# Membrizard/ml_conformer_generator

Hardware: NVIDIA B200
Metric: generated mols/sec (100 EGNN steps + GCN, <=39 atoms) (higher is better)
Workload: dtype fp16

## Files before the change

ml_conformer_generator_b200/csrc/mlcg_api.cu:

```cuda
#include <algorithm>
#include <cstddef>
#include <cstdlib>
#include <cstring>
#include <map>
#include <string>
#include <vector>

#include "mlcg.h"
#include "mlcg_kernels.cuh"
#include "mlcg_tc.cuh"
#include "mlcg_tc3.cuh"
#include "mlcg_shape.cuh"
#include "mlcg_ifm.cuh"

using namespace mlcg;

namespace {

struct Wt {
  float* d = nullptr;
  int rows = 0, cols = 0;
};

struct DevBuf {
// ... 94 lines not shown
#define KCHECK()                                 \
  do {                                           \
    h->launches++;                               \
    CK(cudaGetLastError());                      \
  } while (0)
#define FAIL(code, msg) \
  do {                  \
    h->err = (msg);     \
    return (code);      \
  } while (0)

static thread_local std::string g_create_err;

enum { BD_START = -1, BD_PREPARE = 0, BD_PQ = 1, BD_EDGE_GCL = 2, BD_EDGE_EQUIV = 3, BD_FIXUP = 4, BD_MLP1 = 5, BD_MLP2 = 6,
       BD_READOUT = 7, BD_NCLASS = 8 };
static void bd_mark(mlcg_handle* h, int cls, cudaStream_t st) {
  if (!h->bd_on) return;
  cudaEvent_t e;
  if (cudaEventCreate(&e) != cudaSuccess) return;
  cudaEventRecord(e, st);
  h->bd_ev.emplace_back(cls, e);
}

template <int kMode, int BN, int kEpi>
static cudaError_t launch_gemm(const GemmArgs& a, int n_mtiles, int n_ntiles, cudaStream_t st) {
  static bool attr_set = false;
  if (!attr_set) {
    cudaError_t e = cudaFuncSetAttribute(k_tc_gemm<kMode, BN, kEpi>, cudaFuncAttributeMaxDynamicSharedMemorySize,
                                         GemmCfg<BN>::SMEM_BYTES);
    if (e != cudaSuccess) return e;
    attr_set = true;
  }
  static int num_sms = 0;
  if (num_sms == 0) {
    int dev = 0;
    cudaGetDevice(&dev);
    cudaDeviceGetAttribute(&num_sms, cudaDevAttrMultiProcessorCount, dev);
    if (num_sms <= 0) num_sms = 148;
  }
  GemmArgs b = a;
  b.n_mtiles = n_mtiles;
  b.n_ntiles = n_ntiles;
  k_tc_gemm<kMode, BN, kEpi><<<std::min(n_mtiles * n_ntiles, num_sms), GEMM_THREADS, GemmCfg<BN>::SMEM_BYTES, st>>>(b);
  return cudaGetLastError();
}
template <int BN, int kEpi>
static cudaError_t launch_gemm_mode(int mode, const GemmArgs& a, int n_mtiles, int n_ntiles, cudaStream_t st) {
  if (mode == PREC_FP16) return launch_gemm<PREC_FP16, BN, kEpi>(a, n_mtiles, n_ntiles, st);
  return mode == PREC_BF16 ? launch_gemm<PREC_BF16, BN, kEpi>(a, n_mtiles, n_ntiles, st)
                           : launch_gemm<PREC_TF32, BN, kEpi>(a, n_mtiles, n_ntiles, st);
}
template <int kMode, bool kEquiv, bool kPair, bool kDistF32 = false, bool kProf = false>
static cudaError_t launch_edge(const EdgeArgs& a, int grid, cudaStream_t st) {
  static bool attr_set = false;
  if (!attr_set) {
    cudaError_t e = cudaFuncSetAttribute(k_tc_edge<kMode, kEquiv, kPair, kDistF32, kProf>, cudaFuncAttributeMaxDynamicSharedMemorySize,
                                         EdgeSmemT<kMode>::ALLOC);
    if (e != cudaSuccess) return e;
    attr_set = true;
  }
  cudaLaunchConfig_t cfg{};
  cfg.gridDim = dim3(grid);
  cfg.blockDim = dim3(EDGE_THREADS);
  cfg.dynamicSmemBytes = EdgeSmemT<kMode>::ALLOC;
  cfg.stream = st;
  cudaLaunchAttribute attr[1];
  attr[0].id = cudaLaunchAttributeClusterDimension;
  attr[0].val.clusterDim.x = kPair ? 2 : 1;
  attr[0].val.clusterDim.y = 1;
  attr[0].val.clusterDim.z = 1;
  cfg.attrs = attr;
  cfg.numAttrs = 1;
  return cudaLaunchKernelEx(&cfg, k_tc_edge<kMode, kEquiv, kPair, kDistF32, kProf>, a);
// ... 612 lines not shown
      return (u + 0x7fffu + ((u >> 16) & 1u)) >> 16;
    };
    for (int k2 = 0; k2 < HP / 2; ++k2) {
      a.wcd_h[4 * (k2 / 2) + (k2 & 1)] = bf(L.h_wc[2 * k2]) | (bf(L.h_wc[2 * k2 + 1]) << 16);
      a.wcd_h[4 * (k2 / 2) + 2 + (k2 & 1)] = bf(L.h_wd[2 * k2]) | (bf(L.h_wd[2 * k2 + 1]) << 16);
    }
  }
  a.att_bias = L.att_bias;
  a.agg_op = h->agg_op.as<uint8_t>();
  a.agg_chunks = h->kc448();
  a.prof = nullptr;
  return a;
}

static int egnn_forward_tc(mlcg_handle* h, cudaStream_t st) {
  const int mode = h->precision, kc = h->kc448();
  const int grid_e = edge_grid(h);
  auto gemm_pq = [&](const LayerW& L) -> cudaError_t {
    GemmArgs a{};
    a.a0 = h->h_op.as<uint8_t>(); a.a0_chunks = kc; a.a0_per_tile = kc; a.n_kc = kc;
    a.w = L.w1ab_op.as<uint8_t>(); a.bias = L.bias_pq.as<float>(); a.m_rows = h->pl->M;
    a.out_f32 = h->pq.as<float>(); a.ldo = 2 * HP; a.n_valid = 2 * HP; a.rowscale = nullptr; a.relu = 0;
    a.out_scale = act_scale(mode);
    if (mode == PREC_FP16) return launch_gemm<PREC_FP16, HP, EPI_BF16>(a, h->pl->n_mtiles, 2, st);
    if (mode == PREC_BF16) return launch_gemm<PREC_BF16, HP, EPI_BF16>(a, h->pl->n_mtiles, 2, st);
    return launch_gemm<PREC_TF32, HP, EPI_F32>(a, h->pl->n_mtiles, 2, st);
  };
  float* xa = h->xa.as<float>();
  float* xb = h->xb.as<float>();
  CK(gemm_pq(h->layers[0]));
  h->launches++;
  bd_mark(h, BD_PQ, st);
  for (int l = 0; l < 27; ++l) {
    const LayerW& L = h->layers[l];
    const int blk = l / 3;
    const float* x_cur = (blk & 1) ? xb : xa;
    float* x_next = (blk & 1) ? xa : xb;
    EdgeArgs ea = edge_args(h, L, x_cur, x_next);
    CK(launch_edge_mode(mode, L.equiv, ea, grid_e, st));
    h->launches++;
    bd_mark(h, L.equiv ? BD_EDGE_EQUIV : BD_EDGE_GCL, st);
    CK(launch_edge_fixup(h, mode, L.equiv, ea, st));
    bd_mark(h, BD_FIXUP, st);
    if (!L.equiv) {
      GemmArgs a{};
      a.a0 = h->h_op.as<uint8_t>(); a.a0_chunks = kc; a.a0_per_tile = kc;
      a.a1 = h->agg_op.as<uint8_t>(); a.a1_per_tile = kc; a.n_kc = 2 * kc;
      a.w = L.w3_op.as<uint8_t>(); a.bias = L.b3p.as<float>(); a.m_rows = h->pl->M;
      a.out_op = h->t_op.as<uint8_t>(); a.out_op_chunks = kc; a.out_scale = op_scale(mode);
      CK((launch_gemm_mode<HP, EPI_SILU_OP>(mode, a, h->pl->n_mtiles, 1, st)));
      h->launches++;
      bd_mark(h, BD_MLP1, st);
      GemmArgs b{};
      b.a0 = h->t_op.as<uint8_t>(); b.a0_chunks = kc; b.a0_per_tile = kc; b.n_kc = kc;
      b.w = L.w4_op.as<uint8_t>(); b.bias = L.b4p.as<float>(); b.m_rows = h->pl->M;
      b.out_op = h->h_op.as<uint8_t>(); b.out_op_chunks = kc; b.resid = h->h_res.as<float>(); b.ldr = 0;
      b.out_scale = op_scale(mode);
      CK((launch_gemm_mode<HP, EPI_RESID_OP>(mode, b, h->pl->n_mtiles, 1, st)));
      h->launches++;
      bd_mark(h, BD_MLP2, st);
    }
    if (l + 1 < 27) {
      CK(gemm_pq(h->layers[l + 1]));
      h->launches++;
      bd_mark(h, BD_PQ, st);
    }
  }
  return MLCG_OK;
}

static int simt_gemm(mlcg_handle* h, const float* A, int lda, const float* W, int ldw, const float* bias, float* C, int ldc,
                     int M, int N, int K, int flags, const float* rowscale, cudaStream_t st) {
  if (M <= 0) return MLCG_OK;
  dim3 grid((N + 63) / 64, (M + 63) / 64);
  k_simt_gemm<<<grid, 256, 0, st>>>(A, lda, W, ldw, bias, rowscale, C, ldc, M, N, K, flags);
  KCHECK();
  return MLCG_OK;
}

static int egnn_forward_simt(mlcg_handle* h, cudaStream_t st) {
  float* xa = h->xa.as<float>();
// ... 704 lines not shown
  KCHECK();
  return MLCG_OK;
}

extern "C" int mlcg_ifm_merge_inputs(mlcg_handle* h, const float* x_gen, const int32_t* cls_gen, const float* shift,
                                     const float* rot, const float* ff_x, const float* ff_h, int n_ff, int B, int Ng, int N,
                                     float* z_known, float* fixed_mask, void* stream) {
  if (!h) return MLCG_E_ARG;
  if (!x_gen || !cls_gen || !shift || !rot || !ff_x || !ff_h || !z_known || !fixed_mask || B <= 0 || n_ff <= 0 || Ng <= 0 ||
      N < n_ff || N > 64)
    FAIL(MLCG_E_ARG, "ifm_merge_inputs: bad argument");
  k_ifm_merge_inputs<<<B, 64, 0, (cudaStream_t)stream>>>(x_gen, cls_gen, shift, rot, ff_x, ff_h, n_ff, Ng, N, z_known, fixed_mask);
  KCHECK();
  return MLCG_OK;
}

extern "C" int mlcg_gemm_phase_profile(mlcg_handle* h, int which, double* out, void* stream) {
  if (!h || !out) return MLCG_E_ARG;
  if (!h->egnn_loaded || !h->batch_set || h->precision == PREC_FP32_SIMT || which < 0 || which > 2)
    FAIL(MLCG_E_STATE, "gemm_phase_profile: needs a tensor-core precision, weights, a batch and which in 0..2");
  cudaStream_t st = (cudaStream_t)stream;
  const int mode = h->precision, kc = h->kc448();
  const LayerW& L = h->layers[0];
  const int grid = std::min(h->pl->n_mtiles * (which == 0 ? 2 : 1), h->num_sms);
  DevBuf buf;
  CK(buf.ensure((size_t)grid * 8 * sizeof(long long)));
  CK(cudaMemsetAsync(buf.p, 0, (size_t)grid * 8 * sizeof(long long), st));
  GemmArgs a{};
  a.prof = buf.as<long long>();
  a.m_rows = h->pl->M;
  a.out_scale = (which == 0) ? act_scale(mode) : op_scale(mode);
  cudaEvent_t e0, e1;
  CK(cudaEventCreate(&e0));
  CK(cudaEventCreate(&e1));
  CK(cudaEventRecord(e0, st));
  if (which == 0) {
    a.a0 = h->h_op.as<uint8_t>(); a.a0_chunks = kc; a.a0_per_tile = kc; a.n_kc = kc;
    a.w = L.w1ab_op.as<uint8_t>(); a.bias = L.bias_pq.as<float>();
    a.out_f32 = h->pq.as<float>(); a.ldo = 2 * HP; a.n_valid = 2 * HP;
    if (mode == PREC_FP16) CK((launch_gemm<PREC_FP16, HP, EPI_BF16>(a, h->pl->n_mtiles, 2, st)));
    else if (mode == PREC_BF16) CK((launch_gemm<PREC_BF16, HP, EPI_BF16>(a, h->pl->n_mtiles, 2, st)));
    else CK((launch_gemm<PREC_TF32, HP, EPI_F32>(a, h->pl->n_mtiles, 2, st)));
  } else if (which == 1) {
    a.a0 = h->h_op.as<uint8_t>(); a.a0_chunks = kc; a.a0_per_tile = kc;
    a.a1 = h->agg_op.as<uint8_t>(); a.a1_per_tile = kc; a.n_kc = 2 * kc;
    a.w = L.w3_op.as<uint8_t>(); a.bias = L.b3p.as<float>();
    a.out_op = h->t_op.as<uint8_t>(); a.out_op_chunks = kc;
    CK((launch_gemm_mode<HP, EPI_SILU_OP>(mode, a, h->pl->n_mtiles, 1, st)));
  } else {
    a.a0 = h->t_op.as<uint8_t>(); a.a0_chunks = kc; a.a0_per_tile = kc; a.n_kc = kc;
    a.w = L.w4_op.as<uint8_t>(); a.bias = L.b4p.as<float>();
    a.out_op = h->h_op.as<uint8_t>(); a.out_op_chunks = kc; a.resid = h->h_res.as<float>(); a.ldr = 0;
    CK((launch_gemm_mode<HP, EPI_RESID_OP>(mode, a, h->pl->n_mtiles, 1, st)));
  }
  CK(cudaEventRecord(e1, st));
  h->launches++;
  std::vector<long long> host((size_t)grid * 8);
  CK(cudaMemcpyAsync(host.data(), buf.p, host.size() * sizeof(long long), cudaMemcpyDeviceToHost, st));
  CK(cudaStreamSynchronize(st));
  float ms = 0.f;
  cudaEventElapsedTime(&ms, e0, e1);
  cudaEventDestroy(e0);
  cudaEventDestroy(e1);
  buf.release();
  for (int k = 0; k < 8; ++k) out[k] = 0.0;
  for (int b = 0; b < grid; ++b)
    for (int k = 0; k < 7; ++k) out[k] += (double)host[(size_t)b * 8 + k] / grid;
  out[7] = ms;
  return MLCG_OK;
}

extern "C" int mlcg_test_gemm(mlcg_handle* h, int mode, int bn, const float* a, const float* w, const float* bias, float* c,
                              int M, int N, int K, void* stream) {
  if (!h) return MLCG_E_ARG;
  if ((mode != PREC_TF32 && mode != PREC_BF16 && mode != PREC_FP16) || (bn != 448 && bn != 256) || !a || !w || !bias || !c || M <= 0 || N <= 0 || K <= 0)
    FAIL(MLCG_E_ARG, "test_gemm: bad argument");
  if (N % 4 != 0) FAIL(MLCG_E_ARG, "test_gemm: N must be a multiple of 4");
  cudaStream_t st = (cudaStream_t)stream;
  const int kc = (K + epc(mode) - 1) / epc(mode);
  const int mt = (M + TILE_M - 1) / TILE_M, nt = (N + bn - 1) / bn;
  CK(h->tg_a.ensure((size_t)mt * kc * A_CHUNK_BYTES));
  CK(h->tg_w.ensure((size_t)nt * kc * bn * CHUNK_BYTES));
  CK(h->tg_b.ensure((size_t)nt * bn * 4));
  CK(cudaMemsetAsync(h->tg_b.p, 0, (size_t)nt * bn * 4, st));
  CK(cudaMemcpyAsync(h->tg_b.p, bias, (size_t)N * 4, cudaMemcpyDeviceToDevice, st));
  const long long pieces = (long long)M * kc * 8;
  if (mode == PREC_FP16) k_rowmajor_to_op<PREC_FP16><<<(unsigned)((pieces + 255) / 256), 256, 0, st>>>(a, K, M, K, h->tg_a.as<uint8_t>(), kc);
  else if (mode == PREC_BF16) k_rowmajor_to_op<PREC_BF16><<<(unsigned)((pieces + 255) / 256), 256, 0, st>>>(a, K, M, K, h->tg_a.as<uint8_t>(), kc);
  else k_rowmajor_to_op<PREC_TF32><<<(unsigned)((pieces + 255) / 256), 256, 0, st>>>(a, K, M, K, h->tg_a.as<uint8_t>(), kc);
  KCHECK();
  PackArgs pa{};
  pa.src = w; pa.ld = K; pa.n_real = N; pa.bn = bn; pa.n_kc = kc; pa.seg_len = kc * epc(mode); pa.kreal0 = K;
  pa.bias = nullptr; pa.bias_k = -1; pa.dst = h->tg_w.as<uint8_t>();
  CK(launch_pack(mode, pa, nt, st));
  h->launches++;
  GemmArgs g{};
  g.a0 = h->tg_a.as<uint8_t>(); g.a0_chunks = kc; g.a0_per_tile = kc; g.n_kc = kc;
  g.w = h->tg_w.as<uint8_t>(); g.bias = h->tg_b.as<float>(); g.m_rows = M;
  g.out_f32 = c; g.ldo = N; g.n_valid = N; g.rowscale = nullptr; g.relu = 0;
  if (bn == 448) CK((launch_gemm_mode<448, EPI_F32>(mode, g, mt, nt, st)));
  else CK((launch_gemm_mode<256, EPI_F32>(mode, g, mt, nt, st)));
  h->launches++;
  return MLCG_OK;
}
```

ml_conformer_generator_b200/csrc/mlcg_tc.cuh:

```cuda
#pragma once
#include "mlcg_common.cuh"

namespace mlcg {

enum GemmEpi { EPI_F32 = 0, EPI_SILU_OP = 1, EPI_RESID_OP = 2, EPI_BF16 = 3 };

struct GemmArgs {
  const uint8_t* a0;
  const uint8_t* a1;
  int a0_chunks;
  int a0_per_tile;
  int a1_per_tile;
  int n_kc;
  const uint8_t* w;
  const float* bias;
  int m_rows;
  float* out_f32;
  int ldo;
  int n_valid;
  const float* rowscale;
  int relu;
  uint8_t* out_op;
  int out_op_chunks;
  float* resid;
  int ldr;
  float out_scale;
  int n_mtiles, n_ntiles;
  long long* prof;
};

template <int BN>
struct GemmCfg {
  static constexpr int NSTAGE = (BN == 448) ? 3 : 4;
  static constexpr int NPER = (BN == 448) ? 224 : BN;
  static constexpr int NH = BN / NPER;
  static constexpr int STAGE_BYTES = A_CHUNK_BYTES + BN * CHUNK_BYTES;
  static constexpr int TMEM_COLS = (BN > 256) ? 512 : 256;
  static constexpr int BIAS_OFF = NSTAGE * STAGE_BYTES + 256;
  static constexpr int SMEM_BYTES = NSTAGE * STAGE_BYTES + 1024  + 256  + 2 * BN * 4;
};

#ifndef MLCG_GEMM_NSUB
#define MLCG_GEMM_NSUB 2
#endif
constexpr int GEMM_NSUB = MLCG_GEMM_NSUB;
constexpr int GEMM_THREADS = 64 + 128 * GEMM_NSUB;

template <int kMode, int BN, int kEpi>
__global__ void __launch_bounds__(GEMM_THREADS, 1) k_tc_gemm(const GemmArgs p) {
  using Cfg = GemmCfg<BN>;
  constexpr bool kFast = is16(kMode);
  extern __shared__ uint8_t smem_raw[];
  const uint32_t base = (smem_u32(smem_raw) + 1023u) & ~1023u;
  uint8_t* gen_base = smem_raw + (base - smem_u32(smem_raw));
  const uint32_t bar0 = base + Cfg::NSTAGE * Cfg::STAGE_BYTES;
  auto full_bar = [&](int s) { return bar0 + 8u * s; };
  auto empty_bar = [&](int s) { return bar0 + 8u * (Cfg::NSTAGE + s); };
  const uint32_t dfull_bar = bar0 + 8u * (2 * Cfg::NSTAGE);
  uint32_t* tmem_slot = reinterpret_cast<uint32_t*>(gen_base + Cfg::NSTAGE * Cfg::STAGE_BYTES + 8 * (2 * Cfg::NSTAGE + 2));

  const uint32_t epi_done = dfull_bar + 8u;
  const int warp = threadIdx.x >> 5, lane = threadIdx.x & 31;
  const int n_tiles = p.n_mtiles * p.n_ntiles;

  if (threadIdx.x == 0) {
    for (int s = 0; s < Cfg::NSTAGE; ++s) {
      mbar_init(full_bar(s), 1);
      mbar_init(empty_bar(s), 1);
    }
    mbar_init(dfull_bar, 1);
    mbar_init(epi_done, 4 * GEMM_NSUB);
    fence_barrier_init();
  }
  if (warp == 1) tmem_alloc<Cfg::TMEM_COLS>(smem_u32(tmem_slot));
// ... 67 lines not shown
#pragma unroll
            for (int ks = 0; ks < 4; ++ks)
              umma<kMode>(tmem_base + nh * Cfg::NPER, adesc + 2 * ks, bdesc + 2 * ks, idesc, (kc | ks) != 0);
          }
          umma_commit(empty_bar(sl));
        }
        umma_commit(dfull_bar);
      }
      if (p.prof) {
        p.prof[(size_t)blockIdx.x * 8 + 1] = w_ops;
        p.prof[(size_t)blockIdx.x * 8 + 2] = w_epi;
        p.prof[(size_t)blockIdx.x * 8 + 5] = tl;
        p.prof[(size_t)blockIdx.x * 8 + 6] = clock64() - t_start;
      }
    }
  } else {
   int tl = 0;
   long long w_acc = 0, t_epi = 0;
   for (int tile = blockIdx.x; tile < n_tiles; tile += gridDim.x, ++tl) {
    const int mt = tile / p.n_ntiles, nt = tile - mt * p.n_ntiles;
    float* bias_s = reinterpret_cast<float*>(gen_base + Cfg::BIAS_OFF) + (tl & 1) * BN;
    for (int i = threadIdx.x - 64; i < BN; i += GEMM_THREADS - 64) bias_s[i] = p.bias[nt * BN + i];
    named_bar_sync(1, GEMM_THREADS - 64);
    const int q = warp & 3;
    const int row = q * 32 + lane;
    const int grow = mt * TILE_M + row;
    const bool rvalid = grow < p.m_rows;
    const long long pc0 = p.prof ? clock64() : 0;
    mbar_wait(dfull_bar, (uint32_t)(tl & 1));
    tc_fence_after();
    const long long pc1 = p.prof ? clock64() : 0;
    const uint32_t trow = tmem_base + ((uint32_t)(q * 32) << 16);
    if constexpr (kEpi == EPI_F32) {
      float rs = 1.0f;
      if (p.rowscale != nullptr && rvalid) rs = p.rowscale[grow];
      for (int c0 = ((warp - 2) >> 2) * 32; c0 < BN; c0 += 32 * GEMM_NSUB) {
        float v[32];
        tmem_ld32(trow + c0, v);
        tmem_wait_ld();
        const int gcol = nt * BN + c0;
        if (rvalid) {
          const float4* b4 = reinterpret_cast<const float4*>(bias_s + c0);
          float* orow = p.out_f32 + (size_t)grow * p.ldo + gcol;
#pragma unroll
          for (int e = 0; e < 32; e += 4) {
            const float4 b = b4[e >> 2];
            float4 o;
            o.x = fmaf(rs, b.x, v[e + 0]);
            o.y = fmaf(rs, b.y, v[e + 1]);
            o.z = fmaf(rs, b.z, v[e + 2]);
            o.w = fmaf(rs, b.w, v[e + 3]);
            if (p.relu) {
              o.x = fmaxf(o.x, 0.f); o.y = fmaxf(o.y, 0.f); o.z = fmaxf(o.z, 0.f); o.w = fmaxf(o.w, 0.f);
            }
            if (gcol + e + 3 < p.n_valid) {
              *reinterpret_cast<float4*>(orow + e) = o;
            } else {
              if (gcol + e + 0 < p.n_valid) orow[e + 0] = o.x;
              if (gcol + e + 1 < p.n_valid) orow[e + 1] = o.y;
              if (gcol + e + 2 < p.n_valid) orow[e + 2] = o.z;
            }
          }
        }
      }
    } else {
      constexpr int EPC = epc(kMode);
      constexpr int UNIT = EPC / 32;
      constexpr int NBLK = BN / EPC;
      const int sub = (warp - 2) >> 2;
      const int n_my = ((NBLK - sub + GEMM_NSUB - 1) / GEMM_NSUB) * UNIT;
      auto group_c0 = [&](int k) { return ((sub + GEMM_NSUB * (k / UNIT)) * UNIT + (k % UNIT)) * 32; };
      uint8_t* stg = gen_base + (sub * 4 + q) * 4096;
      const int crow = lane >> 3, cpiece = lane & 7;
      auto stg_at = [&](int r, int pc) { return stg + r * 128 + ((pc ^ (r & 7)) << 4); };
      const int row0 = mt * TILE_M + q * 32;
      uint32_t ow[32];
      [[maybe_unused]] uint4 rnext[8];
      if constexpr (kEpi == EPI_RESID_OP) {
        if (n_my > 0) {
          const uint4* nblk = reinterpret_cast<const uint4*>(p.resid + hres_index(row0, nt * BN + group_c0(0), 0));
#pragma unroll
          for (int i = 0; i < 8; ++i) rnext[i] = nblk[i * 32 + lane];
        }
      }
      for (int gk = 0; gk < n_my; ++gk) {
        const int c0 = group_c0(gk);
        float v[32];
        tmem_ld32(trow + c0, v);
        tmem_wait_ld();
        const int gcol = nt * BN + c0;
        const float4* b4 = reinterpret_cast<const float4*>(bias_s + c0);
        if constexpr (kEpi == EPI_RESID_OP) {
          float* rblk = p.resid + hres_index(row0, gcol, 0);
#pragma unroll
          for (int i = 0; i < 8; ++i) *reinterpret_cast<uint4*>(stg_at(4 * i + crow, cpiece)) = rnext[i];
          if (gk + 1 < n_my) {
            const uint4* nblk = reinterpret_cast<const uint4*>(p.resid + hres_index(row0, nt * BN + group_c0(gk + 1), 0));
#pragma unroll
            for (int i = 0; i < 8; ++i) rnext[i] = nblk[i * 32 + lane];
          }
          __syncwarp();
#pragma unroll
          for (int e = 0; e < 32; e += 4) {
            const float4 b = b4[e >> 2];
            float4 h = *reinterpret_cast<const float4*>(stg_at(lane, e >> 2));
            h.x += v[e + 0] + b.x;
            h.y += v[e + 1] + b.y;
            h.z += v[e + 2] + b.z;
            h.w += v[e + 3] + b.w;
            *reinterpret_cast<float4*>(stg_at(lane, e >> 2)) = h;
            v[e + 0] = h.x; v[e + 1] = h.y; v[e + 2] = h.z; v[e + 3] = h.w;
          }
          __syncwarp();
#pragma unroll
          for (int i = 0; i < 8; ++i)
            if (row0 + 4 * i + crow < p.m_rows)
              reinterpret_cast<uint4*>(rblk)[i * 32 + lane] = *reinterpret_cast<const uint4*>(stg_at(4 * i + crow, cpiece));
          __syncwarp();
        } else {
#pragma unroll
          for (int e = 0; e < 32; e += 4) {
            const float4 b = b4[e >> 2];
            if constexpr (kEpi == EPI_SILU_OP) {
              v[e + 0] = silu<kFast>(v[e + 0] + b.x); v[e + 1] = silu<kFast>(v[e + 1] + b.y);
              v[e + 2] = silu<kFast>(v[e + 2] + b.z); v[e + 3] = silu<kFast>(v[e + 3] + b.w);
            } else {
              v[e + 0] += b.x; v[e + 1] += b.y; v[e + 2] += b.z; v[e + 3] += b.w;
            }
          }
        }
        if constexpr (kMode == PREC_FP16) {
#pragma unroll
          for (int e = 0; e < 32; ++e) v[e] *= p.out_scale;
        }
        const bool flush = (EPC == 32) || ((c0 & 32) != 0);
        if constexpr (EPC == 32) {
#pragma unroll
          for (int j = 0; j < 32; ++j) ow[j] = f32_to_tf32(v[j]);
        } else {
          if ((c0 & 32) == 0) {
#pragma unroll
            for (int j = 0; j < 16; ++j) ow[j] = pack_h2<kMode>(v[2 * j], v[2 * j + 1]);
          } else {
#pragma unroll
            for (int j = 0; j < 16; ++j) ow[16 + j] = pack_h2<kMode>(v[2 * j], v[2 * j + 1]);
          }
        }
        if (flush) {
#pragma unroll
          for (int pc = 0; pc < 8; ++pc)
            *reinterpret_cast<uint4*>(stg_at(lane, pc)) = make_uint4(ow[4 * pc], ow[4 * pc + 1], ow[4 * pc + 2], ow[4 * pc + 3]);
          __syncwarp();
          const int cb0 = nt * BN + (c0 / EPC) * EPC;
          if constexpr (kEpi == EPI_BF16) {
            uint8_t* obase = reinterpret_cast<uint8_t*>(p.out_f32) + (size_t)cb0 * 2 + cpiece * 16;
#pragma unroll
            for (int i = 0; i < 8; ++i) {
              const int r = 4 * i + crow;
              if (row0 + r < p.m_rows)
                *reinterpret_cast<uint4*>(obase + (size_t)(row0 + r) * p.ldo * 2) = *reinterpret_cast<const uint4*>(stg_at(r, cpiece));
            }
          } else {
            uint8_t* dst = p.out_op + ((size_t)mt * p.out_op_chunks + cb0 / EPC) * A_CHUNK_BYTES + q * 4096;
#pragma unroll
            for (int i = 0; i < 8; ++i)
              if (row0 + 4 * i + crow < p.m_rows)
                reinterpret_cast<uint4*>(dst)[i * 32 + lane] = reinterpret_cast<const uint4*>(stg)[i * 32 + lane];
          }
          __syncwarp();
        }
      }
    }
    tc_fence_before();
    __syncwarp();
    if (lane == 0) mbar_arrive(epi_done);
    if (p.prof) { w_acc += pc1 - pc0; t_epi += clock64() - pc1; }
   }
   if (p.prof && warp == 2 && lane == 0) {
     p.prof[(size_t)blockIdx.x * 8 + 3] = w_acc;
     p.prof[(size_t)blockIdx.x * 8 + 4] = t_epi;
   }
  }
  tc_fence_before();
  __syncthreads();
  if (warp == 1) tmem_dealloc<Cfg::TMEM_COLS>(tmem_base);
}

constexpr int EDGE_MAXG = 12;
constexpr int EDGE_MAXN = 39;
constexpr int EDGE_WSLOT = 224 * CHUNK_BYTES;
constexpr int EDGE_NW = 3;
constexpr int EDGE_NWMAX = EDGE_NW;
constexpr int EDGE_NA = 2;
#ifndef MLCG_EDGE_EARLY
#define MLCG_EDGE_EARLY 2
// ... 762 lines not shown
```

ml_conformer_generator_b200/csrc/mlcg_tc3.cuh:

```cuda
#pragma once
#include <type_traits>
#include <utility>
#include "mlcg_tc.cuh"

namespace mlcg {

constexpr int E3_NT = 144;
constexpr int E3_NKC = 7;
constexpr int E3_DCOL0 = 224;
constexpr int E3_WSLOT = 72 * CHUNK_BYTES;
constexpr int E3_NW_GCL = 5;
constexpr int E3_NW_EQ = 16;
constexpr int E3_EARLY = 2;

template <int kMode, bool kEquiv>
struct Edge3Smem {
  static constexpr int E3_NW = kEquiv ? E3_NW_EQ : E3_NW_GCL;
  static constexpr int NSTG = kEquiv ? 0 : 7;
  static constexpr int PQ_PITCH = 912;
  static constexpr int PQ_ROW = HP * 2;
  static constexpr int W_OFF = 0;
  static constexpr int STG_OFF = W_OFF + E3_NW * E3_WSLOT;
  static constexpr int SEL_OFF = STG_OFF + NSTG * A_CHUNK_BYTES;
  static constexpr int Q_OFF = SEL_OFF + 2 * 4096;
// ... 705 lines not shown
                if (cin) val = carry_rd[ch] + val;
                if (cout) carry_wr[ch] = val;
                else if (fx >= 0) atomicAdd(p.fix_agg + (size_t)fx * HP + ch, val);
                else store_h<kMode>(gdst + (size_t)cb * 2 * A_CHUNK_BYTES, val * agg_out_scale(kMode));
              }
            }
          }
        }
      }
      tick(12);
      named_bar_sync(1, EDGE_CT);
      tick(13);
      if (profiling) pacc[6] += 1;
    }
    if (profiling)
      for (int k = 0; k < 14; ++k) p.prof[(size_t)blockIdx.x * 16 + k] = pacc[k];
  }
  tc_fence_before();
  __syncthreads();
  cluster_sync_all();
  if (warp == 1) tmem_dealloc_pair<512>(tmem_base);
}

}
```

Measured before the change: 819.6.

## Add 2-CTA cluster tensor-core GEMM for 448-wide 16-bit projections

Adds a new GEMM kernel that runs as a 2-CTA cluster using paired UMMA (M=256). Each CTA loads only half of the weight tile, and the output is split into 256- and 192-column accumulators that are double-buffered in TMEM, so epilogue and MMA can overlap. The shared epilogue is factored out of k_tc_gemm and reused. PQ, MLP1 and MLP2 in the EGNN loop now use this kernel in fp16/bf16 mode. The aim is to halve weight traffic per CTA and improve tensor-core utilization, at the cost of cluster synchronization, odd-tile handling (duplicated mt) and fewer independent CTAs.

```diff
diff --git a/ml_conformer_generator_b200/csrc/mlcg_api.cu b/ml_conformer_generator_b200/csrc/mlcg_api.cu
--- a/ml_conformer_generator_b200/csrc/mlcg_api.cu
+++ b/ml_conformer_generator_b200/csrc/mlcg_api.cu
@@ -140,6 +140,16 @@
   h->bd_ev.emplace_back(cls, e);
 }
 
+static int gemm_num_sms() {
+  static int num_sms = 0;
+  if (num_sms == 0) {
+    int dev = 0;
+    cudaGetDevice(&dev);
+    cudaDeviceGetAttribute(&num_sms, cudaDevAttrMultiProcessorCount, dev);
+    if (num_sms <= 0) num_sms = 148;
+  }
+  return num_sms;
+}
 template <int kMode, int BN, int kEpi>
 static cudaError_t launch_gemm(const GemmArgs& a, int n_mtiles, int n_ntiles, cudaStream_t st) {
   static bool attr_set = false;
@@ -149,17 +159,10 @@
     if (e != cudaSuccess) return e;
     attr_set = true;
   }
-  static int num_sms = 0;
-  if (num_sms == 0) {
-    int dev = 0;
-    cudaGetDevice(&dev);
-    cudaDeviceGetAttribute(&num_sms, cudaDevAttrMultiProcessorCount, dev);
-    if (num_sms <= 0) num_sms = 148;
-  }
   GemmArgs b = a;
   b.n_mtiles = n_mtiles;
   b.n_ntiles = n_ntiles;
-  k_tc_gemm<kMode, BN, kEpi><<<std::min(n_mtiles * n_ntiles, num_sms), GEMM_THREADS, GemmCfg<BN>::SMEM_BYTES, st>>>(b);
+  k_tc_gemm<kMode, BN, kEpi><<<std::min(n_mtiles * n_ntiles, gemm_num_sms()), GEMM_THREADS, GemmCfg<BN>::SMEM_BYTES, st>>>(b);
   return cudaGetLastError();
 }
 template <int BN, int kEpi>
@@ -167,6 +170,43 @@
   if (mode == PREC_FP16) return launch_gemm<PREC_FP16, BN, kEpi>(a, n_mtiles, n_ntiles, st);
   return mode == PREC_BF16 ? launch_gemm<PREC_BF16, BN, kEpi>(a, n_mtiles, n_ntiles, st)
                            : launch_gemm<PREC_TF32, BN, kEpi>(a, n_mtiles, n_ntiles, st);
+}
+static int gemm_pair_grid(int n_mtiles, int n_packs) {
+  const int n_pt = ((n_mtiles + 1) / 2) * 2 * n_packs;
+  return 2 * std::max(1, std::min(n_pt, gemm_num_sms() / 2));
+}
+template <int kMode, int kEpi>
+static cudaError_t launch_gemm_pair(const GemmArgs& a, int n_mtiles, int n_packs, cudaStream_t st) {
+  static bool attr_set = false;
+  if (!attr_set) {
+    cudaError_t e = cudaFuncSetAttribute(k_tc_gemm_pair<kMode, kEpi>, cudaFuncAttributeMaxDynamicSharedMemorySize,
+                                         GemmPairSmem::ALLOC);
+    if (e != cudaSuccess) return e;
+    attr_set = true;
+  }
+  GemmArgs b = a;
+  b.n_mtiles = n_mtiles;
+  b.n_ntiles = n_packs;
+  cudaLaunchConfig_t cfg{};
+  cfg.gridDim = dim3(gemm_pair_grid(n_mtiles, n_packs));
+  cfg.blockDim = dim3(GEMM_THREADS);
+  cfg.dynamicSmemBytes = GemmPairSmem::ALLOC;
+  cfg.stream = st;
+  cudaLaunchAttribute attr[1];
+  attr[0].id = cudaLaunchAttributeClusterDimension;
+  attr[0].val.clusterDim.x = 2;
+  attr[0].val.clusterDim.y = 1;
+  attr[0].val.clusterDim.z = 1;
+  cfg.attrs = attr;
+  cfg.numAttrs = 1;
+  return cudaLaunchKernelEx(&cfg, k_tc_gemm_pair<kMode, kEpi>, b);
+}
+template <int kEpi>
+static cudaError_t launch_gemm448(int mode, const GemmArgs& a, int n_mtiles, int n_packs, cudaStream_t st) {
+  if (mode == PREC_FP16) return launch_gemm_pair<PREC_FP16, kEpi>(a, n_mtiles, n_packs, st);
+  if (mode == PREC_BF16) return launch_gemm_pair<PREC_BF16, kEpi>(a, n_mtiles, n_packs, st);
+  if constexpr (kEpi == EPI_BF16) return cudaErrorInvalidValue;
+  else return launch_gemm<PREC_TF32, HP, kEpi>(a, n_mtiles, n_packs, st);
 }
 template <int kMode, bool kEquiv, bool kPair, bool kDistF32 = false, bool kProf = false>
 static cudaError_t launch_edge(const EdgeArgs& a, int grid, cudaStream_t st) {
@@ -825,8 +865,7 @@
     a.w = L.w1ab_op.as<uint8_t>(); a.bias = L.bias_pq.as<float>(); a.m_rows = h->pl->M;
     a.out_f32 = h->pq.as<float>(); a.ldo = 2 * HP; a.n_valid = 2 * HP; a.rowscale = nullptr; a.relu = 0;
     a.out_scale = act_scale(mode);
-    if (mode == PREC_FP16) return launch_gemm<PREC_FP16, HP, EPI_BF16>(a, h->pl->n_mtiles, 2, st);
-    if (mode == PREC_BF16) return launch_gemm<PREC_BF16, HP, EPI_BF16>(a, h->pl->n_mtiles, 2, st);
+    if (is16(mode)) return launch_gemm448<EPI_BF16>(mode, a, h->pl->n_mtiles, 2, st);
     return launch_gemm<PREC_TF32, HP, EPI_F32>(a, h->pl->n_mtiles, 2, st);
   };
   float* xa = h->xa.as<float>();
@@ -851,7 +890,7 @@
       a.a1 = h->agg_op.as<uint8_t>(); a.a1_per_tile = kc; a.n_kc = 2 * kc;
       a.w = L.w3_op.as<uint8_t>(); a.bias = L.b3p.as<float>(); a.m_rows = h->pl->M;
       a.out_op = h->t_op.as<uint8_t>(); a.out_op_chunks = kc; a.out_scale = op_scale(mode);
-      CK((launch_gemm_mode<HP, EPI_SILU_OP>(mode, a, h->pl->n_mtiles, 1, st)));
+      CK((launch_gemm448<EPI_SILU_OP>(mode, a, h->pl->n_mtiles, 1, st)));
       h->launches++;
       bd_mark(h, BD_MLP1, st);
       GemmArgs b{};
@@ -859,7 +898,7 @@
       b.w = L.w4_op.as<uint8_t>(); b.bias = L.b4p.as<float>(); b.m_rows = h->pl->M;
       b.out_op = h->h_op.as<uint8_t>(); b.out_op_chunks = kc; b.resid = h->h_res.as<float>(); b.ldr = 0;
       b.out_scale = op_scale(mode);
-      CK((launch_gemm_mode<HP, EPI_RESID_OP>(mode, b, h->pl->n_mtiles, 1, st)));
+      CK((launch_gemm448<EPI_RESID_OP>(mode, b, h->pl->n_mtiles, 1, st)));
       h->launches++;
       bd_mark(h, BD_MLP2, st);
     }
@@ -1610,7 +1649,9 @@
   cudaStream_t st = (cudaStream_t)stream;
   const int mode = h->precision, kc = h->kc448();
   const LayerW& L = h->layers[0];
-  const int grid = std::min(h->pl->n_mtiles * (which == 0 ? 2 : 1), h->num_sms);
+  const int n_packs = which == 0 ? 2 : 1;
+  const bool pair = is16(mode);
+  const int grid = pair ? gemm_pair_grid(h->pl->n_mtiles, n_packs) : std::min(h->pl->n_mtiles * n_packs, h->num_sms);
   DevBuf buf;
   CK(buf.ensure((size_t)grid * 8 * sizeof(long long)));
   CK(cudaMemsetAsync(buf.p, 0, (size_t)grid * 8 * sizeof(long long), st));
@@ -1626,20 +1667,19 @@
     a.a0 = h->h_op.as<uint8_t>(); a.a0_chunks = kc; a.a0_per_tile = kc; a.n_kc = kc;
     a.w = L.w1ab_op.as<uint8_t>(); a.bias = L.bias_pq.as<float>();
     a.out_f32 = h->pq.as<float>(); a.ldo = 2 * HP; a.n_valid = 2 * HP;
-    if (mode == PREC_FP16) CK((launch_gemm<PREC_FP16, HP, EPI_BF16>(a, h->pl->n_mtiles, 2, st)));
-    else if (mode == PREC_BF16) CK((launch_gemm<PREC_BF16, HP, EPI_BF16>(a, h->pl->n_mtiles, 2, st)));
+    if (is16(mode)) CK((launch_gemm448<EPI_BF16>(mode, a, h->pl->n_mtiles, 2, st)));
     else CK((launch_gemm<PREC_TF32, HP, EPI_F32>(a, h->pl->n_mtiles, 2, st)));
   } else if (which == 1) {
     a.a0 = h->h_op.as<uint8_t>(); a.a0_chunks = kc; a.a0_per_tile = kc;
     a.a1 = h->agg_op.as<uint8_t>(); a.a1_per_tile = kc; a.n_kc = 2 * kc;
     a.w = L.w3_op.as<uint8_t>(); a.bias = L.b3p.as<float>();
     a.out_op = h->t_op.as<uint8_t>(); a.out_op_chunks = kc;
-    CK((launch_gemm_mode<HP, EPI_SILU_OP>(mode, a, h->pl->n_mtiles, 1, st)));
+    CK((launch_gemm448<EPI_SILU_OP>(mode, a, h->pl->n_mtiles, 1, st)));
   } else {
     a.a0 = h->t_op.as<uint8_t>(); a.a0_chunks = kc; a.a0_per_tile = kc; a.n_kc = kc;
     a.w = L.w4_op.as<uint8_t>(); a.bias = L.b4p.as<float>();
     a.out_op = h->h_op.as<uint8_t>(); a.out_op_chunks = kc; a.resid = h->h_res.as<float>(); a.ldr = 0;
-    CK((launch_gemm_mode<HP, EPI_RESID_OP>(mode, a, h->pl->n_mtiles, 1, st)));
+    CK((launch_gemm448<EPI_RESID_OP>(mode, a, h->pl->n_mtiles, 1, st)));
   }
   CK(cudaEventRecord(e1, st));
   h->launches++;
@@ -1653,7 +1693,11 @@
   buf.release();
   for (int k = 0; k < 8; ++k) out[k] = 0.0;
   for (int b = 0; b < grid; ++b)
-    for (int k = 0; k < 7; ++k) out[k] += (double)host[(size_t)b * 8 + k] / grid;
+    for (int k = 0; k < 7; ++k) {
+      const bool leader_only = pair && (k == 1 || k == 2);
+      if (!leader_only) out[k] += (double)host[(size_t)b * 8 + k] / grid;
+      else if (b % 2 == 0) out[k] += (double)host[(size_t)b * 8 + k] / (grid / 2);
+    }
   out[7] = ms;
   return MLCG_OK;
 }
@@ -1686,7 +1730,7 @@
   g.a0 = h->tg_a.as<uint8_t>(); g.a0_chunks = kc; g.a0_per_tile = kc; g.n_kc = kc;
   g.w = h->tg_w.as<uint8_t>(); g.bias = h->tg_b.as<float>(); g.m_rows = M;
   g.out_f32 = c; g.ldo = N; g.n_valid = N; g.rowscale = nullptr; g.relu = 0;
-  if (bn == 448) CK((launch_gemm_mode<448, EPI_F32>(mode, g, mt, nt, st)));
+  if (bn == 448) CK((launch_gemm448<EPI_F32>(mode, g, mt, nt, st)));
   else CK((launch_gemm_mode<256, EPI_F32>(mode, g, mt, nt, st)));
   h->launches++;
   return MLCG_OK;
diff --git a/ml_conformer_generator_b200/csrc/mlcg_tc.cuh b/ml_conformer_generator_b200/csrc/mlcg_tc.cuh
--- a/ml_conformer_generator_b200/csrc/mlcg_tc.cuh
+++ b/ml_conformer_generator_b200/csrc/mlcg_tc.cuh
@@ -46,10 +46,152 @@
 constexpr int GEMM_NSUB = MLCG_GEMM_NSUB;
 constexpr int GEMM_THREADS = 64 + 128 * GEMM_NSUB;
 
+__device__ __forceinline__ int sub_of(int warp) { return (warp - 2) >> 2; }
+template <int kMode, int kEpi>
+__device__ __forceinline__ void gemm_epilogue(const GemmArgs& p, uint32_t tacc, int width, int gcol0, int mt, const float* bias_s,
+                                              uint8_t* stg_area, int warp, int lane) {
+  constexpr bool kFast = is16(kMode);
+  const int q = warp & 3;
+  const int row = q * 32 + lane;
+  const int grow = mt * TILE_M + row;
+  const bool rvalid = grow < p.m_rows;
+  const uint32_t trow = tacc + ((uint32_t)(q * 32) << 16);
+  if constexpr (kEpi == EPI_F32) {
+    float rs = 1.0f;
+    if (p.rowscale != nullptr && rvalid) rs = p.rowscale[grow];
+    for (int c0 = sub_of(warp) * 32; c0 < width; c0 += 32 * GEMM_NSUB) {
+      float v[32];
+      tmem_ld32(trow + c0, v);
+      tmem_wait_ld();
+      const int gcol = gcol0 + c0;
+      if (rvalid) {
+        const float4* b4 = reinterpret_cast<const float4*>(bias_s + c0);
+        float* orow = p.out_f32 + (size_t)grow * p.ldo + gcol;
+#pragma unroll
+        for (int e = 0; e < 32; e += 4) {
+          const float4 b = b4[e >> 2];
+          float4 o;
+          o.x = fmaf(rs, b.x, v[e + 0]);
+          o.y = fmaf(rs, b.y, v[e + 1]);
+          o.z = fmaf(rs, b.z, v[e + 2]);
+          o.w = fmaf(rs, b.w, v[e + 3]);
+          if (p.relu) {
+            o.x = fmaxf(o.x, 0.f); o.y = fmaxf(o.y, 0.f); o.z = fmaxf(o.z, 0.f); o.w = fmaxf(o.w, 0.f);
+          }
+          if (gcol + e + 3 < p.n_valid) {
+            *reinterpret_cast<float4*>(orow + e) = o;
+          } else {
+            if (gcol + e + 0 < p.n_valid) orow[e + 0] = o.x;
+            if (gcol + e + 1 < p.n_valid) orow[e + 1] = o.y;
+            if (gcol + e + 2 < p.n_valid) orow[e + 2] = o.z;
+          }
+        }
+      }
+    }
+  } else {
+    constexpr int EPC = epc(kMode);
+    constexpr int UNIT = EPC / 32;
+    const int NBLK = width / EPC;
+    const int sub = sub_of(warp);
+    const int n_my = ((NBLK - sub + GEMM_NSUB - 1) / GEMM_NSUB) * UNIT;
+    auto group_c0 = [&](int k) { return ((sub + GEMM_NSUB * (k / UNIT)) * UNIT + (k % UNIT)) * 32; };
+    uint8_t* stg = stg_area + (sub * 4 + q) * 4096;
+    const int crow = lane >> 3, cpiece = lane & 7;
+    auto stg_at = [&](int r, int pc) { return stg + r * 128 + ((pc ^ (r & 7)) << 4); };
+    const int row0 = mt * TILE_M + q * 32;
+    uint32_t ow[32];
+    [[maybe_unused]] float4 rnext[8];
+    if constexpr (kEpi == EPI_RESID_OP) {
+      if (n_my > 0) {
+        const float4* nline = reinterpret_cast<const float4*>(p.resid + hres_index(grow, gcol0 + group_c0(0), 0));
+#pragma unroll
+        for (int i = 0; i < 8; ++i) rnext[i] = nline[i];
+      }
+    }
+    for (int gk = 0; gk < n_my; ++gk) {
+      const int c0 = group_c0(gk);
+      float v[32];
+      tmem_ld32(trow + c0, v);
+      tmem_wait_ld();
+      const int gcol = gcol0 + c0;
+      const float4* b4 = reinterpret_cast<const float4*>(bias_s + c0);
+      if constexpr (kEpi == EPI_RESID_OP) {
+        float4* rline = reinterpret_cast<float4*>(p.resid + hres_index(grow, gcol, 0));
+#pragma unroll
+        for (int e = 0; e < 32; e += 4) {
+          const float4 b = b4[e >> 2];
+          float4 h = rnext[e >> 2];
+          h.x += v[e + 0] + b.x;
+          h.y += v[e + 1] + b.y;
+          h.z += v[e + 2] + b.z;
+          h.w += v[e + 3] + b.w;
+          if (rvalid) rline[e >> 2] = h;
+          v[e + 0] = h.x; v[e + 1] = h.y; v[e + 2] = h.z; v[e + 3] = h.w;
+        }
+        if (gk + 1 < n_my) {
+          const float4* nline = reinterpret_cast<const float4*>(p.resid + hres_index(grow, gcol0 + group_c0(gk + 1), 0));
+#pragma unroll
+          for (int i = 0; i < 8; ++i) rnext[i] = nline[i];
+        }
+      } else {
+#pragma unroll
+        for (int e = 0; e < 32; e += 4) {
+          const float4 b = b4[e >> 2];
+          if constexpr (kEpi == EPI_SILU_OP) {
+            v[e + 0] = silu<kFast>(v[e + 0] + b.x); v[e + 1] = silu<kFast>(v[e + 1] + b.y);
+            v[e + 2] = silu<kFast>(v[e + 2] + b.z); v[e + 3] = silu<kFast>(v[e + 3] + b.w);
+          } else {
+            v[e + 0] += b.x; v[e + 1] += b.y; v[e + 2] += b.z; v[e + 3] += b.w;
+          }
+        }
+      }
+      if constexpr (kMode == PREC_FP16) {
+#pragma unroll
+        for (int e = 0; e < 32; ++e) v[e] *= p.out_scale;
+      }
+      const bool flush = (EPC == 32) || ((c0 & 32) != 0);
+      if constexpr (EPC == 32) {
+#pragma unroll
+        for (int j = 0; j < 32; ++j) ow[j] = f32_to_tf32(v[j]);
+      } else {
+        if ((c0 & 32) == 0) {
+#pragma unroll
+          for (int j = 0; j < 16; ++j) ow[j] = pack_h2<kMode>(v[2 * j], v[2 * j + 1]);
+        } else {
+#pragma unroll
+          for (int j = 0; j < 16; ++j) ow[16 + j] = pack_h2<kMode>(v[2 * j], v[2 * j + 1]);
+        }
+      }
+      if (flush) {
+#pragma unroll
+        for (int pc = 0; pc < 8; ++pc)
+          *reinterpret_cast<uint4*>(stg_at(lane, pc)) = make_uint4(ow[4 * pc], ow[4 * pc + 1], ow[4 * pc + 2], ow[4 * pc + 3]);
+        __syncwarp();
+        const int cb0 = gcol0 + (c0 / EPC) * EPC;
+        if constexpr (kEpi == EPI_BF16) {
+          uint8_t* obase = reinterpret_cast<uint8_t*>(p.out_f32) + (size_t)cb0 * 2 + cpiece * 16;
+#pragma unroll
+          for (int i = 0; i < 8; ++i) {
+            const int r = 4 * i + crow;
+            if (row0 + r < p.m_rows)
+              *reinterpret_cast<uint4*>(obase + (size_t)(row0 + r) * p.ldo * 2) = *reinterpret_cast<const uint4*>(stg_at(r, cpiece));
+          }
+        } else {
+          uint8_t* dst = p.out_op + ((size_t)mt * p.out_op_chunks + cb0 / EPC) * A_CHUNK_BYTES + q * 4096;
+#pragma unroll
+          for (int i = 0; i < 8; ++i)
+            if (row0 + 4 * i + crow < p.m_rows)
+              reinterpret_cast<uint4*>(dst)[i * 32 + lane] = reinterpret_cast<const uint4*>(stg)[i * 32 + lane];
+        }
+        __syncwarp();
+      }
+    }
+  }
+}
+
 template <int kMode, int BN, int kEpi>
 __global__ void __launch_bounds__(GEMM_THREADS, 1) k_tc_gemm(const GemmArgs p) {
   using Cfg = GemmCfg<BN>;
-  constexpr bool kFast = is16(kMode);
   extern __shared__ uint8_t smem_raw[];
   const uint32_t base = (smem_u32(smem_raw) + 1023u) & ~1023u;
   uint8_t* gen_base = smem_raw + (base - smem_u32(smem_raw));
@@ -163,155 +305,11 @@
     float* bias_s = reinterpret_cast<float*>(gen_base + Cfg::BIAS_OFF) + (tl & 1) * BN;
     for (int i = threadIdx.x - 64; i < BN; i += GEMM_THREADS - 64) bias_s[i] = p.bias[nt * BN + i];
     named_bar_sync(1, GEMM_THREADS - 64);
-    const int q = warp & 3;
-    const int row = q * 32 + lane;
-    const int grow = mt * TILE_M + row;
-    const bool rvalid = grow < p.m_rows;
     const long long pc0 = p.prof ? clock64() : 0;
     mbar_wait(dfull_bar, (uint32_t)(tl & 1));
     tc_fence_after();
     const long long pc1 = p.prof ? clock64() : 0;
-    const uint32_t trow = tmem_base + ((uint32_t)(q * 32) << 16);
-    if constexpr (kEpi == EPI_F32) {
-      float rs = 1.0f;
-      if (p.rowscale != nullptr && rvalid) rs = p.rowscale[grow];
-      for (int c0 = ((warp - 2) >> 2) * 32; c0 < BN; c0 += 32 * GEMM_NSUB) {
-        float v[32];
-        tmem_ld32(trow + c0, v);
-        tmem_wait_ld();
-        const int gcol = nt * BN + c0;
-        if (rvalid) {
-          const float4* b4 = reinterpret_cast<const float4*>(bias_s + c0);
-          float* orow = p.out_f32 + (size_t)grow * p.ldo + gcol;
-#pragma unroll
-          for (int e = 0; e < 32; e += 4) {
-            const float4 b = b4[e >> 2];
-            float4 o;
-            o.x = fmaf(rs, b.x, v[e + 0]);
-            o.y = fmaf(rs, b.y, v[e + 1]);
-            o.z = fmaf(rs, b.z, v[e + 2]);
-            o.w = fmaf(rs, b.w, v[e + 3]);
-            if (p.relu) {
-              o.x = fmaxf(o.x, 0.f); o.y = fmaxf(o.y, 0.f); o.z = fmaxf(o.z, 0.f); o.w = fmaxf(o.w, 0.f);
-            }
-            if (gcol + e + 3 < p.n_valid) {
-              *reinterpret_cast<float4*>(orow + e) = o;
-            } else {
-              if (gcol + e + 0 < p.n_valid) orow[e + 0] = o.x;
-              if (gcol + e + 1 < p.n_valid) orow[e + 1] = o.y;
-              if (gcol + e + 2 < p.n_valid) orow[e + 2] = o.z;
-            }
-          }
-        }
-      }
-    } else {
-      constexpr int EPC = epc(kMode);
-      constexpr int UNIT = EPC / 32;
-      constexpr int NBLK = BN / EPC;
-      const int sub = (warp - 2) >> 2;
-      const int n_my = ((NBLK - sub + GEMM_NSUB - 1) / GEMM_NSUB) * UNIT;
-      auto group_c0 = [&](int k) { return ((sub + GEMM_NSUB * (k / UNIT)) * UNIT + (k % UNIT)) * 32; };
-      uint8_t* stg = gen_base + (sub * 4 + q) * 4096;
-      const int crow = lane >> 3, cpiece = lane & 7;
-      auto stg_at = [&](int r, int pc) { return stg + r * 128 + ((pc ^ (r & 7)) << 4); };
-      const int row0 = mt * TILE_M + q * 32;
-      uint32_t ow[32];
-      [[maybe_unused]] uint4 rnext[8];
-      if constexpr (kEpi == EPI_RESID_OP) {
-        if (n_my > 0) {
-          const uint4* nblk = reinterpret_cast<const uint4*>(p.resid + hres_index(row0, nt * BN + group_c0(0), 0));
-#pragma unroll
-          for (int i = 0; i < 8; ++i) rnext[i] = nblk[i * 32 + lane];
-        }
-      }
-      for (int gk = 0; gk < n_my; ++gk) {
-        const int c0 = group_c0(gk);
-        float v[32];
-        tmem_ld32(trow + c0, v);
-        tmem_wait_ld();
-        const int gcol = nt * BN + c0;
-        const float4* b4 = reinterpret_cast<const float4*>(bias_s + c0);
-        if constexpr (kEpi == EPI_RESID_OP) {
-          float* rblk = p.resid + hres_index(row0, gcol, 0);
-#pragma unroll
-          for (int i = 0; i < 8; ++i) *reinterpret_cast<uint4*>(stg_at(4 * i + crow, cpiece)) = rnext[i];
-          if (gk + 1 < n_my) {
-            const uint4* nblk = reinterpret_cast<const uint4*>(p.resid + hres_index(row0, nt * BN + group_c0(gk + 1), 0));
-#pragma unroll
-            for (int i = 0; i < 8; ++i) rnext[i] = nblk[i * 32 + lane];
-          }
-          __syncwarp();
-#pragma unroll
-          for (int e = 0; e < 32; e += 4) {
-            const float4 b = b4[e >> 2];
-            float4 h = *reinterpret_cast<const float4*>(stg_at(lane, e >> 2));
-            h.x += v[e + 0] + b.x;
-            h.y += v[e + 1] + b.y;
-            h.z += v[e + 2] + b.z;
-            h.w += v[e + 3] + b.w;
-            *reinterpret_cast<float4*>(stg_at(lane, e >> 2)) = h;
-            v[e + 0] = h.x; v[e + 1] = h.y; v[e + 2] = h.z; v[e + 3] = h.w;
-          }
-          __syncwarp();
-#pragma unroll
-          for (int i = 0; i < 8; ++i)
-            if (row0 + 4 * i + crow < p.m_rows)
-              reinterpret_cast<uint4*>(rblk)[i * 32 + lane] = *reinterpret_cast<const uint4*>(stg_at(4 * i + crow, cpiece));
-          __syncwarp();
-        } else {
-#pragma unroll
-          for (int e = 0; e < 32; e += 4) {
-            const float4 b = b4[e >> 2];
-            if constexpr (kEpi == EPI_SILU_OP) {
-              v[e + 0] = silu<kFast>(v[e + 0] + b.x); v[e + 1] = silu<kFast>(v[e + 1] + b.y);
-              v[e + 2] = silu<kFast>(v[e + 2] + b.z); v[e + 3] = silu<kFast>(v[e + 3] + b.w);
-            } else {
-              v[e + 0] += b.x; v[e + 1] += b.y; v[e + 2] += b.z; v[e + 3] += b.w;
-            }
-          }
-        }
-        if constexpr (kMode == PREC_FP16) {
-#pragma unroll
-          for (int e = 0; e < 32; ++e) v[e] *= p.out_scale;
-        }
-        const bool flush = (EPC == 32) || ((c0 & 32) != 0);
-        if constexpr (EPC == 32) {
-#pragma unroll
-          for (int j = 0; j < 32; ++j) ow[j] = f32_to_tf32(v[j]);
-        } else {
-          if ((c0 & 32) == 0) {
-#pragma unroll
-            for (int j = 0; j < 16; ++j) ow[j] = pack_h2<kMode>(v[2 * j], v[2 * j + 1]);
-          } else {
-#pragma unroll
-            for (int j = 0; j < 16; ++j) ow[16 + j] = pack_h2<kMode>(v[2 * j], v[2 * j + 1]);
-          }
-        }
-        if (flush) {
-#pragma unroll
-          for (int pc = 0; pc < 8; ++pc)
-            *reinterpret_cast<uint4*>(stg_at(lane, pc)) = make_uint4(ow[4 * pc], ow[4 * pc + 1], ow[4 * pc + 2], ow[4 * pc + 3]);
-          __syncwarp();
-          const int cb0 = nt * BN + (c0 / EPC) * EPC;
-          if constexpr (kEpi == EPI_BF16) {
-            uint8_t* obase = reinterpret_cast<uint8_t*>(p.out_f32) + (size_t)cb0 * 2 + cpiece * 16;
-#pragma unroll
-            for (int i = 0; i < 8; ++i) {
-              const int r = 4 * i + crow;
-              if (row0 + r < p.m_rows)
-                *reinterpret_cast<uint4*>(obase + (size_t)(row0 + r) * p.ldo * 2) = *reinterpret_cast<const uint4*>(stg_at(r, cpiece));
-            }
-          } else {
-            uint8_t* dst = p.out_op + ((size_t)mt * p.out_op_chunks + cb0 / EPC) * A_CHUNK_BYTES + q * 4096;
-#pragma unroll
-            for (int i = 0; i < 8; ++i)
-              if (row0 + 4 * i + crow < p.m_rows)
-                reinterpret_cast<uint4*>(dst)[i * 32 + lane] = reinterpret_cast<const uint4*>(stg)[i * 32 + lane];
-          }
-          __syncwarp();
-        }
-      }
-    }
+    gemm_epilogue<kMode, kEpi>(p, tmem_base, BN, nt * BN, mt, bias_s, gen_base, warp, lane);
     tc_fence_before();
     __syncwarp();
     if (lane == 0) mbar_arrive(epi_done);
diff --git a/ml_conformer_generator_b200/csrc/mlcg_tc3.cuh b/ml_conformer_generator_b200/csrc/mlcg_tc3.cuh
--- a/ml_conformer_generator_b200/csrc/mlcg_tc3.cuh
+++ b/ml_conformer_generator_b200/csrc/mlcg_tc3.cuh
@@ -751,4 +751,157 @@
   if (warp == 1) tmem_dealloc_pair<512>(tmem_base);
 }
 
-}
+constexpr int GP_NSTAGE = 5;
+constexpr int GP_STAGE = A_CHUNK_BYTES + 128 * CHUNK_BYTES;
+constexpr int GP_ACC = 256;
+__host__ __device__ constexpr int gp_width(int half) { return half ? HP - GP_ACC : GP_ACC; }
+struct GemmPairSmem {
+  static constexpr int STG_OFF = GP_NSTAGE * GP_STAGE;
+  static constexpr int BIAS_OFF = STG_OFF + 4 * GEMM_NSUB * 4096;
+  static constexpr int BAR_OFF = BIAS_OFF + 2 * GP_ACC * 4;
+  static constexpr int FULL = 0, EMPTY = GP_NSTAGE, D_FULL = 2 * GP_NSTAGE, ACC_EMPTY = 2 * GP_NSTAGE + 2,
+                       TMEM_SLOT = 2 * GP_NSTAGE + 4;
+  static constexpr int ALLOC = BAR_OFF + 8 * (TMEM_SLOT + 1) + 1024;
+  static_assert(ALLOC <= 232448, "shared memory budget");
+};
+
+template <int kMode, int kEpi>
+__global__ void __launch_bounds__(GEMM_THREADS, 1) k_tc_gemm_pair(const GemmArgs p) {
+  static_assert(is16(kMode), "k_tc_gemm_pair serves the 16-bit tensor-core modes");
+  using S = GemmPairSmem;
+  extern __shared__ uint8_t smem_raw[];
+  const uint32_t base = (smem_u32(smem_raw) + 1023u) & ~1023u;
+  uint8_t* gen_base = smem_raw + (base - smem_u32(smem_raw));
+  const uint32_t bar0 = base + S::BAR_OFF;
+  auto full_bar = [&](int s) { return bar0 + 8u * (S::FULL + s); };
+  auto empty_bar = [&](int s) { return bar0 + 8u * (S::EMPTY + s); };
+  auto d_full = [&](int a) { return bar0 + 8u * (S::D_FULL + a); };
+  auto acc_empty = [&](int a) { return bar0 + 8u * (S::ACC_EMPTY + a); };
+  uint32_t* tmem_slot = reinterpret_cast<uint32_t*>(gen_base + S::BAR_OFF + 8 * S::TMEM_SLOT);
+  const int warp = __shfl_sync(0xffffffffu, (int)(threadIdx.x >> 5), 0), lane = threadIdx.x & 31;
+  const uint32_t crank = (uint32_t)__shfl_sync(0xffffffffu, (int)cluster_ctarank(), 0);
+  const int cluster = blockIdx.x >> 1, n_clusters = gridDim.x >> 1;
+  const int n_sub = 2 * p.n_ntiles;
+  const int n_pt = ((p.n_mtiles + 1) >> 1) * n_sub;
+  constexpr int NEPI = 4 * GEMM_NSUB;
+
+  if (threadIdx.x == 0) {
+    for (int s = 0; s < GP_NSTAGE; ++s) {
+      mbar_init(full_bar(s), crank == 0 ? 3 : 2);
+      mbar_init(empty_bar(s), 1);
+    }
+    for (int a = 0; a < 2; ++a) {
+      mbar_init(d_full(a), 1);
+      mbar_init(acc_empty(a), 2 * NEPI);
+    }
+    fence_barrier_init();
+  }
+  if (warp == 1) tmem_alloc_pair<512>(smem_u32(tmem_slot));
+  tc_fence_before();
+  __syncthreads();
+  cluster_sync_all();
+  tc_fence_after();
+  const uint32_t tmem_base = *tmem_slot;
+
+  if (warp == 0) {
+    uint32_t sl = 0, ph = 1;
+    long long w_slot = 0;
+    for (int pt = cluster; pt < n_pt; pt += n_clusters) {
+      const int mp = pt / n_sub, sub = pt - mp * n_sub, nt = sub >> 1, half = sub & 1;
+      int mt = 2 * mp + (int)crank;
+      if (mt >= p.n_mtiles) mt -= 1;
+      const uint32_t w_half = (uint32_t)(gp_width(half) / 2) * CHUNK_BYTES;
+      const uint8_t* wt = p.w + (size_t)nt * p.n_kc * (HP * CHUNK_BYTES) + (size_t)(half * GP_ACC) * CHUNK_BYTES + crank * w_half;
+      for (int kc = 0; kc < p.n_kc; ++kc) {
+        const long long c0 = p.prof ? clock64() : 0;
+        mbar_wait_lean_w(empty_bar(sl), ph);
+        if (p.prof) w_slot += clock64() - c0;
+        const uint8_t* asrc = (kc < p.a0_chunks)
+                                  ? p.a0 + ((size_t)mt * p.a0_per_tile + kc) * A_CHUNK_BYTES
+                                  : p.a1 + ((size_t)mt * p.a1_per_tile + (kc - p.a0_chunks)) * A_CHUNK_BYTES;
+        const uint32_t sa = base + sl * GP_STAGE;
+        bulk_g2s_expect_e(sa, asrc, A_CHUNK_BYTES, full_bar(sl));
+        bulk_g2s_expect_e(sa + A_CHUNK_BYTES, wt + (size_t)kc * (HP * CHUNK_BYTES), w_half, full_bar(sl));
+        if (++sl == GP_NSTAGE) { sl = 0; ph ^= 1u; }
+      }
+    }
+    if (p.prof && lane == 0) p.prof[(size_t)blockIdx.x * 8 + 0] = w_slot;
+  } else if (warp == 1) {
+    const long long t_start = p.prof ? clock64() : 0;
+    uint32_t sl = 0, ph = 0;
+    int tl = 0;
+    long long w_ops = 0, w_epi = 0;
+    if (crank == 1) {
+      for (int pt = cluster; pt < n_pt; pt += n_clusters, ++tl)
+        for (int kc = 0; kc < p.n_kc; ++kc) {
+          mbar_wait_lean_w(full_bar(sl), ph);
+          mbar_arrive_cluster_e(mapa(full_bar(sl), 0));
+          if (++sl == GP_NSTAGE) { sl = 0; ph ^= 1u; }
+        }
+    } else {
+      constexpr uint32_t idesc256 = umma_idesc(umma_fmt(kMode), 2 * TILE_M, gp_width(0));
+      constexpr uint32_t idesc192 = umma_idesc(umma_fmt(kMode), 2 * TILE_M, gp_width(1));
+      for (int pt = cluster; pt < n_pt; pt += n_clusters, ++tl) {
+        const int acc = tl & 1, u = tl >> 1;
+        const uint32_t idesc = ((pt % n_sub) & 1) ? idesc192 : idesc256;
+        if (u > 0) {
+          const long long c0 = p.prof ? clock64() : 0;
+          mbar_wait_lean_w(acc_empty(acc), (uint32_t)((u - 1) & 1));
+          tc_fence_after();
+          if (p.prof) w_epi += clock64() - c0;
+        }
+        const uint32_t dcol = tmem_base + acc * GP_ACC;
+        for (int kc = 0; kc < p.n_kc; ++kc) {
+          const long long c1 = p.prof ? clock64() : 0;
+          mbar_wait_lean_w(full_bar(sl), ph);
+          tc_fence_after();
+          if (p.prof) w_ops += clock64() - c1;
+          const uint32_t sa = base + sl * GP_STAGE;
+          const uint64_t adesc = umma_desc_sw128(sa), bdesc = umma_desc_sw128(sa + A_CHUNK_BYTES);
+#pragma unroll
+          for (int ks = 0; ks < 4; ++ks) umma_ss_pair_e(dcol, adesc + 2 * ks, bdesc + 2 * ks, idesc, (kc | ks) != 0);
+          umma_commit_pair_e(empty_bar(sl), 3);
+          if (++sl == GP_NSTAGE) { sl = 0; ph ^= 1u; }
+        }
+        umma_commit_pair_e(d_full(acc), 3);
+      }
+    }
+    if (p.prof && lane == 0) {
+      p.prof[(size_t)blockIdx.x * 8 + 1] = w_ops;
+      p.prof[(size_t)blockIdx.x * 8 + 2] = w_epi;
+      p.prof[(size_t)blockIdx.x * 8 + 5] = tl;
+      p.prof[(size_t)blockIdx.x * 8 + 6] = clock64() - t_start;
+    }
+  } else {
+    int tl = 0;
+    long long w_acc = 0, t_epi = 0;
+    for (int pt = cluster; pt < n_pt; pt += n_clusters, ++tl) {
+      const int mp = pt / n_sub, sub = pt - mp * n_sub, half = sub & 1;
+      const int mt = 2 * mp + (int)crank, width = gp_width(half), gcol0 = (sub >> 1) * HP + half * GP_ACC;
+      const int acc = tl & 1;
+      float* bias_s = reinterpret_cast<float*>(gen_base + S::BIAS_OFF) + acc * GP_ACC;
+      for (int i = threadIdx.x - 64; i < width; i += GEMM_THREADS - 64) bias_s[i] = p.bias[gcol0 + i];
+      named_bar_sync(1, GEMM_THREADS - 64);
+      const long long pc0 = p.prof ? clock64() : 0;
+      mbar_wait_lean_w(d_full(acc), (uint32_t)((tl >> 1) & 1));
+      tc_fence_after();
+      const long long pc1 = p.prof ? clock64() : 0;
+      if (mt < p.n_mtiles)
+        gemm_epilogue<kMode, kEpi>(p, tmem_base + acc * GP_ACC, width, gcol0, mt, bias_s, gen_base + S::STG_OFF, warp, lane);
+      tc_fence_before();
+      __syncwarp();
+      if (lane == 0) mbar_arrive_cluster(mapa(acc_empty(acc), 0));
+      if (p.prof) { w_acc += pc1 - pc0; t_epi += clock64() - pc1; }
+    }
+    if (p.prof && warp == 2 && lane == 0) {
+      p.prof[(size_t)blockIdx.x * 8 + 3] = w_acc;
+      p.prof[(size_t)blockIdx.x * 8 + 4] = t_epi;
+    }
+  }
+  tc_fence_before();
+  __syncthreads();
+  cluster_sync_all();
+  if (warp == 1) tmem_dealloc_pair<512>(tmem_base);
+}
+
+}
```

Result: slower. 810.5, median of 6 (-1.1%).
